# GAP-LAB-CUHK-SZ/GaussReg

Hardware: AMD Instinct MI355X
Metric: GS views/sec @1M pts 640x480 (+ radius_neighbors Mpts/sec, see radius_neighbors) (higher is better)
Workload: dtype f32; 1 GPU; diff_gaussian_rasterization forward: 1000000 synthetic Gaussians (SH deg 3), 640x480, 32 views per step per GPU (configs[1]); gaussians=1000000, width=640, height=480, parallelism=per-view sharding x1

## Files before the change

### gaussreg_amd/csrc/rasterizer.hip

```cpp
#include <algorithm>
#include <type_traits>
#include <vector>

#include <atomic>

#include "raster_shared.hpp"

namespace gr {
namespace {

static_assert(TILE == RASTER_TILE, "get_rect / rect_decode (common.hpp) are written for this tile size");


constexpr int KEY_DEPTH_BITS = 27;
constexpr uint32_t KEY_DEPTH_BASE = 0x3E000000u;

__device__ __forceinline__ uint32_t pack_rect(const int* rmin, const int* rmax) {
  const int w = rmax[0] - rmin[0], h = rmax[1] - rmin[1];
  if (w > 63 || h > 63 || rmin[0] > 126 || rmin[1] > 126) return RECT_MARKER26;
  return (uint32_t)rmin[0] | ((uint32_t)rmin[1] << 7) | ((uint32_t)w << 14) | ((uint32_t)h << 20);
}

constexpr int REC_PLANE = 66;
constexpr int SH_ROW = 13;

template <bool HAS_SH, bool HAS_COV, bool SH16, bool LATE>
__global__ __launch_bounds__(256) void preprocess_kernel(
    int P, int D, int M, int V, const DevView* __restrict__ views, const float* __restrict__ means3D,
    const float* __restrict__ shs, const float* __restrict__ colors_precomp,
    const float* __restrict__ opacities, const float* __restrict__ scales,
    const float* __restrict__ rotations, const float* __restrict__ cov3D_precomp, int W, int H,
    int32_t* __restrict__ radii, float4* __restrict__ rec, uint32_t* __restrict__ dfield,
    uint32_t* __restrict__ rect_raw, int32_t* __restrict__ far_flag, DevView cam1, int far_seq,
    int2* __restrict__ key_mm) {
  if (LATE && blockIdx.x == 0 && threadIdx.x < (int)(sizeof(DevView) / 4))
    reinterpret_cast<float*>(const_cast<DevView*>(views))[threadIdx.x] = reinterpret_cast<const float*>(&cam1)[threadIdx.x];
  __shared__ float4 s_sh[(SH16 && !LATE) ? WAVE * SH_ROW : 1];
  __shared__ float4 s_rec[256 / WAVE][4 * REC_PLANE];
  __shared__ int s_mm[2][2][256 / WAVE];
  int i = blockIdx.x * blockDim.x + threadIdx.x;
  float shr[SH16 ? 48 : 1];
  if (SH16 && !LATE) {
    const int g0 = blockIdx.x * 256;
    const int n_here = min(256, P - g0);
    const float4* src = reinterpret_cast<const float4*>(shs + (int64_t)g0 * 48);
#pragma unroll 1
    for (int w = 0; w < 256 / WAVE; ++w) {
      const int lim = min(WAVE, n_here - w * WAVE) * 12;
#pragma unroll
      for (int u = 0; u < 3; ++u) {
        const int f = threadIdx.x + u * 256;
        if (f < lim) {
          const int g = f / 12, j = f - g * 12;
          s_sh[g * SH_ROW + j] = src[w * WAVE * 12 + f];
        }
      }
      __syncthreads();
      if ((int)threadIdx.x / WAVE == w && i < P) {
#pragma unroll
        for (int j = 0; j < 12; ++j) {
          const float4 t = s_sh[(threadIdx.x & (WAVE - 1)) * SH_ROW + j];
          shr[4 * j] = t.x;
          shr[4 * j + 1] = t.y;
          shr[4 * j + 2] = t.z;
          shr[4 * j + 3] = t.w;
        }
      }
      __syncthreads();
    }
  }
  const bool valid = i < P;
  const int lane = threadIdx.x & (WAVE - 1);
  const int wave_first = i - lane;
  i = min(i, P - 1);
  const float p[3] = {means3D[3 * (int64_t)i], means3D[3 * (int64_t)i + 1], means3D[3 * (int64_t)i + 2]};
  const float opacity = opacities[i];
  float c6[6];
  if (HAS_COV) {
#pragma unroll
    for (int k = 0; k < 6; ++k) c6[k] = cov3D_precomp[6 * (int64_t)i + k];
  }
  const int gx = (W + TILE - 1) / TILE, gy = (H + TILE - 1) / TILE;
  const float* sh = HAS_SH ? shs + (int64_t)i * M * 3 : nullptr;
  float cpre[3] = {0.f, 0.f, 0.f};
  if (!HAS_SH) {
#pragma unroll
    for (int k = 0; k < 3; ++k) cpre[k] = colors_precomp[3 * (int64_t)i + k];
  }
  float4* wrec = s_rec[threadIdx.x / WAVE];
  float mod_prev = 0.f;
  bool have_cov = HAS_COV;
  for (int v = 0; v < V; ++v) {
    const DevView& cam = LATE ? cam1 : views[v];
    const int64_t o = (int64_t)v * P + i;
    int out_radius = 0;
    uint32_t out_field = 0u, out_rect = 0u;
    float out_depth = 0.f, out_sxx = INFINITY, out_syy = INFINITY, out_kc = 0.f;
    float2 out_xy = make_float2(0.f, 0.f);
    float4 out_co = make_float4(0.f, 0.f, 0.f, 0.f);
    bool shade = false;
    float rgb[3] = {0.f, 0.f, 0.f};
    float pv[3];
    xform4x3(cam.view, p, pv);
    if (pv[2] > 0.2f) {
      float ph[4];
      xform4x4(cam.proj, p, ph);
      const float pw = 1.0f / (ph[3] + 0.0000001f);
      const float pprojx = ph[0] * pw, pprojy = ph[1] * pw;
      if (!HAS_COV && (!have_cov || cam.scale_mod != mod_prev)) {
        float sc[3], rot[4];
#pragma unroll
        for (int k = 0; k < 3; ++k) sc[k] = scales[3 * (int64_t)i + k];
#pragma unroll
        for (int k = 0; k < 4; ++k) rot[k] = rotations[4 * (int64_t)i + k];
        cov3d_from_scale_rot(sc, cam.scale_mod, rot, c6);
        have_cov = true;
        mod_prev = cam.scale_mod;
      }
      float cv[3];
      cov2d(pv, cam.fx, cam.fy, cam.tanx, cam.tany, c6, cam.view, cv);
      const float det = cv[0] * cv[2] - cv[1] * cv[1];
      if (det != 0.0f) {
        const float det_inv = 1.f / det;
        const float mid = 0.5f * (cv[0] + cv[2]);
        const float sq = sqrtf(fmaxf(0.1f, mid * mid - det));
        const float l1 = mid + sq, l2 = mid - sq;
        const float my_radius = ceilf(3.f * sqrtf(fmaxf(l1, l2)));
        const float px = ((pprojx + 1.0f) * (float)W - 1.0f) * 0.5f;
        const float py = ((pprojy + 1.0f) * (float)H - 1.0f) * 0.5f;
        int rmin[2], rmax[2];
        get_rect(px, py, (int)my_radius, gx, gy, rmin, rmax);
        const int ntile = (rmax[0] - rmin[0]) * (rmax[1] - rmin[1]);
        if (ntile != 0) {
          shade = true;
          if (HAS_SH && SH16 && LATE) {
            const float4* s4 = reinterpret_cast<const float4*>(shs + (int64_t)i * 48);
#pragma unroll
            for (int jj = 0; jj < 12; ++jj) {
              const float4 t4 = s4[jj];
              shr[4 * jj] = t4.x;
              shr[4 * jj + 1] = t4.y;
              shr[4 * jj + 2] = t4.z;
              shr[4 * jj + 3] = t4.w;
            }
            sh_to_rgb(D, p, cam.campos, [&](int k, int c) { return shr[k * 3 + c]; }, rgb);
          }
          out_depth = pv[2];
          out_radius = (int)my_radius;
          out_xy = make_float2(px, py);
          out_co = make_float4(cv[2] * det_inv, -cv[1] * det_inv, cv[0] * det_inv, opacity);
          const bool cullable = det > 0.0f && l2 >= 0.29f && l1 < 1.0e4f;
          const float kc = cullable ? 1.001f / (0.5f / l1 - 2.0e-6f) : INFINITY;
          out_kc = kc;
          if (cullable) {
            out_sxx = 2.0f * cv[0] * 1.004f;
            out_syy = 2.0f * cv[2] * 1.004f;
            const float pcm = __logf(255.0f * opacity) + 2.0e-3f;
            if (pcm > 0.0f) {
              const float cp = pcm + 2.0e-6f * (pcm * kc);
              const float hx = sqrtf(2.0f * cp * cv[0]) * 1.001f + 1.0e-2f;
              const float hy = sqrtf(2.0f * cp * cv[2]) * 1.001f + 1.0e-2f;
              const float xlo = ceilf(px - hx), xhi = floorf(px + hx), ylo = ceilf(py - hy), yhi = floorf(py + hy);
              if (xlo > -1.0e6f && xhi < 1.0e6f && ylo > -1.0e6f && yhi < 1.0e6f) {
                rmin[0] = max(rmin[0], (int)floorf(xlo / (float)TILE));
                rmin[1] = max(rmin[1], (int)floorf(ylo / (float)TILE));
                rmax[0] = min(rmax[0], (int)floorf(xhi / (float)TILE) + 1);
                rmax[1] = min(rmax[1], (int)floorf(yhi / (float)TILE) + 1);
                if (rmax[0] < rmin[0]) rmax[0] = rmin[0];
                if (rmax[1] < rmin[1]) rmax[1] = rmin[1];
              }
            }
          }
          uint32_t dk = __float_as_uint(out_depth) - KEY_DEPTH_BASE;
          if (dk >= (1u << KEY_DEPTH_BITS)) {
            dk = (1u << KEY_DEPTH_BITS) - 1;
            if (LATE) *far_flag = far_seq; else atomicOr(far_flag, 1);
          }
          out_field = dk;
          out_rect = pack_rect(rmin, rmax);
        }
      }
    }
    if (valid) {
      __builtin_nontemporal_store(out_radius, radii + o);
      dfield[o] = out_field;
      rect_raw[o] = out_rect;
    }
    wrec[0 * REC_PLANE + lane] = make_float4(out_xy.x, out_xy.y, out_sxx, out_syy);
    wrec[1 * REC_PLANE + lane] = out_co;
    wrec[3 * REC_PLANE + lane] = make_float4(__int_as_float(out_radius), out_depth, 0.f, 0.f);
    if (key_mm != nullptr) {
      const uint32_t fld = valid ? out_field : 0u;
      const int mn = wave_min_i32_dpp(fld != 0u ? (int)fld : 0x7fffffff), mx = wave_max_i32_dpp((int)fld);
      if (lane == 0) s_mm[v & 1][0][threadIdx.x / WAVE] = mn, s_mm[v & 1][1][threadIdx.x / WAVE] = mx;
      __syncthreads();
      if (threadIdx.x == 0) {
        int bmn = 0x7fffffff, bmx = 0;
#pragma unroll
        for (int w = 0; w < 256 / WAVE; ++w) bmn = min(bmn, s_mm[v & 1][0][w]), bmx = max(bmx, s_mm[v & 1][1][w]);
        key_mm[(int64_t)v * gridDim.x + blockIdx.x] = make_int2(bmn, bmx);
      }
    }
    if (shade && !(HAS_SH && SH16 && LATE)) {
      if (HAS_SH) {
        if (SH16) sh_to_rgb(D, p, cam.campos, [&](int k, int c) { return shr[k * 3 + c]; }, rgb);
        else sh_to_rgb(D, p, cam.campos, [&](int k, int c) { return sh[k * 3 + c]; }, rgb);
      } else {
        rgb[0] = cpre[0]; rgb[1] = cpre[1]; rgb[2] = cpre[2];
      }
    }
    wrec[2 * REC_PLANE + lane] = make_float4(rgb[0], rgb[1], rgb[2], out_kc);
    const unsigned long long vis = __ballot(valid && out_radius > 0);
    __builtin_amdgcn_fence(__ATOMIC_RELEASE, "wavefront");
    __builtin_amdgcn_wave_barrier();
    __builtin_amdgcn_fence(__ATOMIC_ACQUIRE, "wavefront");
    float4* wout = rec + 4 * ((int64_t)v * P + wave_first);
#pragma unroll
    for (int k = 0; k < 4; ++k) {
      const int rl = 16 * k + lane / 4;
      const float4 piece = wrec[(lane & 3) * REC_PLANE + rl];
      if ((vis >> rl) & 1ull) {
        typedef float pre_f4 __attribute__((ext_vector_type(4)));
        __builtin_nontemporal_store(pre_f4{piece.x, piece.y, piece.z, piece.w}, reinterpret_cast<pre_f4*>(wout + 4 * rl + (lane & 3)));
      }
    }
    __builtin_amdgcn_fence(__ATOMIC_RELEASE, "wavefront");
    __builtin_amdgcn_wave_barrier();
    __builtin_amdgcn_fence(__ATOMIC_ACQUIRE, "wavefront");
  }
}

__global__ __launch_bounds__(256) void full_keys_kernel(int64_t n, const float4* __restrict__ rec,
                                                        const int32_t* __restrict__ radii, uint32_t* __restrict__ dfield) {
  const int64_t o = (int64_t)blockIdx.x * blockDim.x + threadIdx.x;
  if (o >= n) return;
  dfield[o] = radii[o] > 0 ? __float_as_uint(rec[4 * o + 3].y) : 0u;
}


__device__ __forceinline__ bool bin_block(int V, int nchunk, int& v, int& c) {
  const int b = blockIdx.x;
  if (V >= 8) {
    const int k = b >> 3;
    v = (b & 7) + 8 * (k / nchunk);
    c = k % nchunk;
    return v < V;
  }
  v = b / nchunk;
  c = b % nchunk;
  return true;
}
inline int bin_grid(int V, int nchunk) { return V >= 8 ? 8 * ((V + 7) / 8) * nchunk : V * nchunk; }
inline bool bin_scans_self(int nchunk, int V) { return !(nchunk <= SCAN_SINGLE_ROW && V <= 4); }
constexpr int SCATTER_WGS = 6;
constexpr int WIDE_T = 1024;

__device__ __forceinline__ constexpr int mod_small(int n, int d) {
  const unsigned long long tab = d <= 4 ? 0x2001'2aab'4001'8001ull : 0x1001'124a'1556'199aull;
  const unsigned int m = (unsigned int)(tab >> (((d - 1) & 3) * 16)) & 0xffffu;
  return n - (int)(((unsigned int)n * m) >> 15) * d;
}
static_assert(mod_small(255, 7) == 255 % 7 && mod_small(254, 3) == 254 % 3 && mod_small(250, 5) == 0 &&
              mod_small(251, 6) == 251 % 6 && mod_small(255, 8) == 7 && mod_small(200, 1) == 0, "mod_small multipliers");
template <typename F>
__device__ __forceinline__ void by_modulus(int mx, F&& f) {
  switch (mx) {
    case 1: f(std::integral_constant<int, 1>{}); break;
    case 2: f(std::integral_constant<int, 2>{}); break;
    case 3: f(std::integral_constant<int, 3>{}); break;
    case 4: f(std::integral_constant<int, 4>{}); break;
    case 5: f(std::integral_constant<int, 5>{}); break;
    case 6: f(std::integral_constant<int, 6>{}); break;
    case 7: f(std::integral_constant<int, 7>{}); break;
    default: f(std::integral_constant<int, 8>{}); break;
  }
}

__global__ __launch_bounds__(BIN_T) void tile_count_kernel(int P, int V, int gx, int gy, int nchunk,
                                                           const int32_t* __restrict__ nvis,
                                                           const uint32_t* __restrict__ rects,
                                                           const int32_t* __restrict__ ids,
                                                           const float4* __restrict__ rec,
                                                           uint16_t* __restrict__ chunk_cnt,
                                                           int32_t* __restrict__ chunk_total) {
  extern __shared__ unsigned int s_hist[];
  __shared__ int s_wsum[BIN_T / WAVE];
  int v, c;
  if (!bin_block(V, nchunk, v, c)) return;
  const int tiles = gx * gy;
  for (int T = threadIdx.x; T < tiles; T += BIN_T) s_hist[T] = 0u;
  __syncthreads();
  const int64_t vbase = (int64_t)v * P;
  const int nv = nvis[v];
  int mine = 0;
  uint32_t rr[BIN_CHUNK / BIN_T];
#pragma unroll
  for (int it = 0; it < BIN_CHUNK / BIN_T; ++it) {
    const int t = c * BIN_CHUNK + it * BIN_T + threadIdx.x;
    rr[it] = t < nv ? rects[vbase + t] : 0u;
  }
#pragma unroll
  for (int it = 0; it < BIN_CHUNK / BIN_T; ++it) {
    const int t = c * BIN_CHUNK + it * BIN_T + threadIdx.x;
    const uint32_t r = rr[it];
    if (r == 0u) continue;
    int x0, y0, w, h;
    if (!rect_decode(r, r == RECT_MARKER26 ? ids[vbase + t] : 0, vbase, rec, gx, gy, x0, y0, w, h)) continue;
    mine += w * h;
    for (int y = y0; y < y0 + h; ++y)
      for (int x = x0; x < x0 + w; ++x) atomicAdd(&s_hist[y * gx + x], 1u);
  }
  const int wsum = wave_sum_i32_dpp(mine);
  if ((threadIdx.x & (WAVE - 1)) == 0) s_wsum[threadIdx.x / WAVE] = wsum;
  __syncthreads();
  uint16_t* dst = chunk_cnt + ((int64_t)v * nchunk + c) * tiles;
  for (int T = threadIdx.x; T < tiles; T += BIN_T) dst[T] = (uint16_t)s_hist[T];
  if (threadIdx.x == 0) {
    int tot = 0;
    for (int i = 0; i < BIN_T / WAVE; ++i) tot += s_wsum[i];
    chunk_total[v * nchunk + c] = tot;
  }
}

__global__ __launch_bounds__(BIN_T) void chunk_total_kernel(int P, int V, int gx, int gy, int nchunk,
                                                            const int32_t* __restrict__ nvis,
                                                            const uint32_t* __restrict__ rects,
                                                            const int32_t* __restrict__ ids,
                                                            const float4* __restrict__ rec,
                                                            int32_t* __restrict__ chunk_total) {
  __shared__ int s_wsum[BIN_T / WAVE];
  int v, c;
  if (!bin_block(V, nchunk, v, c)) return;
  const int64_t vbase = (int64_t)v * P;
  const int nv = nvis[v];
  int mine = 0;
  uint32_t rr[BIN_CHUNK / BIN_T];
#pragma unroll
  for (int it = 0; it < BIN_CHUNK / BIN_T; ++it) {
    const int t = c * BIN_CHUNK + it * BIN_T + threadIdx.x;
    rr[it] = t < nv ? rects[vbase + t] : 0u;
  }
#pragma unroll
  for (int it = 0; it < BIN_CHUNK / BIN_T; ++it) {
    const int t = c * BIN_CHUNK + it * BIN_T + threadIdx.x;
    const uint32_t r = rr[it];
    int x0, y0, w, h;
    if (r != 0u && rect_decode(r, r == RECT_MARKER26 ? ids[vbase + t] : 0, vbase, rec, gx, gy, x0, y0, w, h)) mine += w * h;
  }
  const int wsum = wave_sum_i32_dpp(mine);
  if ((threadIdx.x & (WAVE - 1)) == 0) s_wsum[threadIdx.x / WAVE] = wsum;
  __syncthreads();
  if (threadIdx.x == 0) {
    int tot = 0;
    for (int i = 0; i < BIN_T / WAVE; ++i) tot += s_wsum[i];
    chunk_total[v * nchunk + c] = tot;
  }
}

__global__ __launch_bounds__(1024) void chunk_max_kernel(int n, const int32_t* __restrict__ chunk_total,
                                                         int32_t* __restrict__ chunk_max) {
  __shared__ int s_m[1024 / WAVE];
  int m = 0;
  for (int i = threadIdx.x; i < n; i += 1024) m = max(m, chunk_total[i]);
  m = wave_max_i32_dpp(m);
  if ((threadIdx.x & (WAVE - 1)) == 0) s_m[threadIdx.x / WAVE] = m;
  __syncthreads();
  if (threadIdx.x == 0) {
    for (int i = 0; i < 1024 / WAVE; ++i) m = max(m, s_m[i]);
    *chunk_max = m;
  }
}

template <bool SELF>
__global__ __launch_bounds__(256) void seg_scan_kernel(int V, int tiles, int nchunk, const uint16_t* __restrict__ chunk_cnt,
                                                       const int32_t* __restrict__ chunk_base ,
                                                       int32_t* __restrict__ totals, uint32_t* __restrict__ seg_off,
                                                       int32_t* __restrict__ mail, int mail_seq) {
  __shared__ int s_w[256 / WAVE];
  __shared__ int s_carry;
  const int v = blockIdx.x / nchunk, c = blockIdx.x % nchunk;
  const int lane = threadIdx.x & (WAVE - 1), wv = threadIdx.x / WAVE;
  int vb = 0;
  if (SELF) {
    const int me = (int)blockIdx.x;
    int part = 0;
    for (int i = threadIdx.x; i < me; i += 256) part += chunk_base[i];
    part = wave_sum_i32_dpp(part);
    if (lane == 0) s_w[wv] = part;
    __syncthreads();
    vb = s_w[0] + s_w[1] + s_w[2] + s_w[3];
    __syncthreads();
    if (c == 0) {
      int sum = 0, mx = 0;
      for (int i = threadIdx.x; i < nchunk; i += 256) {
        const int t = chunk_base[v * nchunk + i];
        sum += t;
        mx = max(mx, t);
      }
      sum = wave_sum_i32_dpp(sum);
      mx = wave_max_i32_dpp(mx);
      if (lane == 0) {
        s_w[wv] = sum;
      }
      __shared__ int s_m[256 / WAVE];
      if (lane == 0) s_m[wv] = mx;
      __syncthreads();
      if (threadIdx.x == 0) {
        const int tv = s_w[0] + s_w[1] + s_w[2] + s_w[3], mv = max(max(s_m[0], s_m[1]), max(s_m[2], s_m[3]));
        totals[v] = tv;
        totals[V + v] = mv;
        if (mail != nullptr) {
          __hip_atomic_store(&mail[v], tv, __ATOMIC_RELAXED, __HIP_MEMORY_SCOPE_SYSTEM);
          __hip_atomic_store(&mail[V + v], mv, __ATOMIC_RELAXED, __HIP_MEMORY_SCOPE_SYSTEM);
          if (v == 0) __hip_atomic_store(&mail[2 * V], totals[2 * V], __ATOMIC_RELAXED, __HIP_MEMORY_SCOPE_SYSTEM);
          __hip_atomic_store(&mail[2 * V + 1 + v], mail_seq, __ATOMIC_RELEASE, __HIP_MEMORY_SCOPE_SYSTEM);
        }
      }
      __syncthreads();
    }
  } else {
    for (int u = 0; u < v; ++u) vb += totals[u];
  }
  const uint16_t* src = chunk_cnt + ((int64_t)v * nchunk + c) * tiles;
  uint32_t* dst = seg_off + ((int64_t)v * nchunk + c) * (tiles + 1);
  if (threadIdx.x == 0) s_carry = SELF ? vb : vb + chunk_base[v * nchunk + c];
  __syncthreads();
  for (int T0 = 0; T0 < tiles; T0 += 256) {
    const int T = T0 + threadIdx.x;
    const int n = T < tiles ? (int)src[T] : 0;
    const int incl = wave_incl_scan_add_dpp(n);
    if (lane == WAVE - 1) s_w[wv] = incl;
    __syncthreads();
    int base = s_carry;
    for (int i = 0; i < wv; ++i) base += s_w[i];
    if (T < tiles) dst[T] = (uint32_t)(base + incl - n);
    __syncthreads();
    if (threadIdx.x == 255) s_carry = base + incl;
    __syncthreads();
  }
  if (threadIdx.x == 0) dst[tiles] = (uint32_t)s_carry;
}

constexpr int SEG_READ = 0, SEG_SELF_RAW = 1, SEG_SELF_SCAN = 2;
struct SelfSeg {
  const int32_t* chunk_total;
  int32_t* totals;
  int32_t* mail;
  int mail_seq;
};
template <bool LANE_ORDERED, int TT, int SEG = SEG_READ>
__global__ __launch_bounds__(TT) void tile_scatter_kernel(int P, int V, int gx, int gy, int nchunk, int tile_bits,
                                                             int stage_cap, const int32_t* __restrict__ nvis,
                                                             const uint32_t* __restrict__ rects,
                                                             const int32_t* __restrict__ ids,
                                                             const float4* __restrict__ rec,
                                                             uint32_t* __restrict__ seg_off,
                                                             int32_t* __restrict__ point_list, unsigned int list_cap, int elist_cap,
                                                             SelfSeg self) {
  extern __shared__ unsigned int s_cur[];
  constexpr int NW = TT / WAVE, CW = BIN_CHUNK / NW;
  constexpr bool SELF = SEG != SEG_READ;
  int v, c;
  if (!bin_block(V, nchunk, v, c)) return;
  const int tiles = gx * gy;
  const int row = (tiles + 1) & ~1;
  uint32_t* seg = seg_off + ((int64_t)v * nchunk + c) * (tiles + 1);
  const int lane = threadIdx.x & (WAVE - 1), wv = threadIdx.x / WAVE;
  const int64_t vbase = (int64_t)v * P;
  const int w_begin = c * BIN_CHUNK + wv * (BIN_CHUNK / (TT / WAVE));
  uint32_t rr[BIN_CHUNK / TT];
  int32_t ii[BIN_CHUNK / TT];
#pragma unroll
  for (int j = 0; j < BIN_CHUNK / TT; ++j) {
    const int64_t o = vbase + min(w_begin + j * WAVE + lane, P - 1);
    rr[j] = rects[o];
    ii[j] = ids[o];
  }
  const int nv = nvis[v];
  __shared__ int s_red[2][TT / WAVE];
  __shared__ unsigned int s_carry;
  unsigned int chunk_begin;
  int total;
  if (SEG == SEG_SELF_RAW) {
    const int me = v * nchunk + c;
    int part = 0;
    for (int i = threadIdx.x; i < me; i += TT) part += self.chunk_total[i];
    part = wave_sum_i32_dpp(part);
    if (lane == 0) s_red[0][wv] = part;
    __syncthreads();
    int front = 0;
#pragma unroll
    for (int w2 = 0; w2 < TT / WAVE; ++w2) front += s_red[0][w2];
    chunk_begin = (unsigned int)front;
    total = self.chunk_total[me];
    if (c == 0) {
      __syncthreads();
      int sum = 0, mx = 0;
      for (int i = threadIdx.x; i < nchunk; i += TT) {
        const int t = self.chunk_total[v * nchunk + i];
        sum += t;
        mx = max(mx, t);
      }
      sum = wave_sum_i32_dpp(sum);
      mx = wave_max_i32_dpp(mx);
      if (lane == 0) s_red[0][wv] = sum, s_red[1][wv] = mx;
      __syncthreads();
      if (threadIdx.x == 0) {
        int tv = 0, mv = 0;
        for (int w2 = 0; w2 < TT / WAVE; ++w2) tv += s_red[0][w2], mv = max(mv, s_red[1][w2]);
        self.totals[v] = tv;
        self.totals[V + v] = mv;
        if (self.mail != nullptr) {
          __hip_atomic_store(&self.mail[v], tv, __ATOMIC_RELAXED, __HIP_MEMORY_SCOPE_SYSTEM);
          __hip_atomic_store(&self.mail[V + v], mv, __ATOMIC_RELAXED, __HIP_MEMORY_SCOPE_SYSTEM);
          if (v == 0) __hip_atomic_store(&self.mail[2 * V], self.totals[2 * V], __ATOMIC_RELAXED, __HIP_MEMORY_SCOPE_SYSTEM);
          __hip_atomic_store(&self.mail[2 * V + 1 + v], self.mail_seq, __ATOMIC_RELEASE, __HIP_MEMORY_SCOPE_SYSTEM);
        }
      }
    }
  } else if (SEG == SEG_SELF_SCAN) {
    unsigned int front = (unsigned int)self.chunk_total[(int64_t)V * nchunk + v * nchunk + c];
    for (int u = 0; u < v; ++u) front += (unsigned int)self.totals[u];
    chunk_begin = front;
    total = self.chunk_total[v * nchunk + c];
  } else {
    chunk_begin = seg[0];
// ... 1216 lines not shown
```

Before: 13270 views/s.

## Double-buffer SH staging, hoist covariance, scalar-load camera, shrink record writes

The SH staging loop in preprocess now double-buffers through the s_sh and s_rec shared buffers and prefetches the next slice into registers, which removes one barrier per slice. The 3D covariance is computed once before the view loop for non-LATE paths. The camera is fetched as wide scalar loads pinned to SGPRs. Shared-memory record writes happen only for visible Gaussians, and the store loop batches its LDS reads before the nontemporal global stores. Together these aim to cut barrier stalls, redundant scale/rotation loads and LDS traffic in the per-view loop. The cost is more register pressure and reliance on invisible lanes' stale LDS slots never being written out, which the visibility ballot masks.

```diff
diff --git a/gaussreg_amd/csrc/rasterizer.hip b/gaussreg_amd/csrc/rasterizer.hip
--- a/gaussreg_amd/csrc/rasterizer.hip
+++ b/gaussreg_amd/csrc/rasterizer.hip
@@ -42,32 +42,36 @@
   float shr[SH16 ? 48 : 1];
   if (SH16 && !LATE) {
     const int g0 = blockIdx.x * 256;
-    const int n_here = min(256, P - g0);
+    const int last = min(256, P - g0) * 12 - 1;
     const float4* src = reinterpret_cast<const float4*>(shs + (int64_t)g0 * 48);
-#pragma unroll 1
-    for (int w = 0; w < 256 / WAVE; ++w) {
-      const int lim = min(WAVE, n_here - w * WAVE) * 12;
-#pragma unroll
-      for (int u = 0; u < 3; ++u) {
-        const int f = threadIdx.x + u * 256;
-        if (f < lim) {
-          const int g = f / 12, j = f - g * 12;
-          s_sh[g * SH_ROW + j] = src[w * WAVE * 12 + f];
-        }
+    const int f0 = threadIdx.x, f1 = threadIdx.x + 256, f2 = threadIdx.x + 512;
+    const int d0 = f0 + f0 / 12, d1 = f1 + f1 / 12, d2 = f2 + f2 / 12;
+    float4* const bufa = reinterpret_cast<float4*>(&s_rec[0][0]);
+    float4 r0 = src[min(f0, last)], r1 = src[min(f1, last)], r2 = src[min(f2, last)];
+    auto slice = [&](auto wc) {
+      constexpr int w = decltype(wc)::value;
+      float4* const b = (w & 1) ? s_sh : bufa;
+      b[d0] = r0, b[d1] = r1, b[d2] = r2;
+      if (w + 1 < 256 / WAVE) {
+        const int o = (w + 1) * WAVE * 12;
+        r0 = src[min(o + f0, last)], r1 = src[min(o + f1, last)], r2 = src[min(o + f2, last)];
       }
       __syncthreads();
-      if ((int)threadIdx.x / WAVE == w && i < P) {
+      if ((int)threadIdx.x / WAVE == w) {
 #pragma unroll
         for (int j = 0; j < 12; ++j) {
-          const float4 t = s_sh[(threadIdx.x & (WAVE - 1)) * SH_ROW + j];
+          const float4 t = b[(threadIdx.x & (WAVE - 1)) * SH_ROW + j];
           shr[4 * j] = t.x;
           shr[4 * j + 1] = t.y;
           shr[4 * j + 2] = t.z;
           shr[4 * j + 3] = t.w;
         }
       }
-      __syncthreads();
-    }
+    };
+    slice(std::integral_constant<int, 0>{});
+    slice(std::integral_constant<int, 1>{});
+    slice(std::integral_constant<int, 2>{});
+    slice(std::integral_constant<int, 3>{});
   }
   const bool valid = i < P;
   const int lane = threadIdx.x & (WAVE - 1);
@@ -90,14 +94,37 @@
   float4* wrec = s_rec[threadIdx.x / WAVE];
   float mod_prev = 0.f;
   bool have_cov = HAS_COV;
+  if (!HAS_COV && !LATE) {
+    float sc[3], rot[4];
+#pragma unroll
+    for (int k = 0; k < 3; ++k) sc[k] = scales[3 * (int64_t)i + k];
+#pragma unroll
+    for (int k = 0; k < 4; ++k) rot[k] = rotations[4 * (int64_t)i + k];
+    mod_prev = views[0].scale_mod;
+    cov3d_from_scale_rot(sc, mod_prev, rot, c6);
+    have_cov = true;
+  }
   for (int v = 0; v < V; ++v) {
-    const DevView& cam = LATE ? cam1 : views[v];
+    typedef uint32_t cam_x16 __attribute__((ext_vector_type(16), aligned(4)));
+    typedef uint32_t cam_x8 __attribute__((ext_vector_type(8), aligned(4)));
+    static_assert(offsetof(DevView, bg) == 160, "the camera without bg is fetched as 16 + 16 + 8 words");
+    DevView cam;
+    if (LATE) {
+      cam = cam1;
+    } else {
+      const uint32_t* cw = reinterpret_cast<const uint32_t*>(views + v);
+      cam_x16 c0 = *reinterpret_cast<const cam_x16*>(cw), c1 = *reinterpret_cast<const cam_x16*>(cw + 16);
+      cam_x8 c2 = *reinterpret_cast<const cam_x8*>(cw + 32);
+      asm volatile("" : "+s"(c0), "+s"(c1), "+s"(c2));
+#pragma unroll
+      for (int k = 0; k < 16; ++k) cam.view[k] = __uint_as_float(c0[k]), cam.proj[k] = __uint_as_float(c1[k]);
+      cam.campos[0] = __uint_as_float(c2[0]), cam.campos[1] = __uint_as_float(c2[1]), cam.campos[2] = __uint_as_float(c2[2]);
+      cam.tanx = __uint_as_float(c2[3]), cam.tany = __uint_as_float(c2[4]);
+      cam.fx = __uint_as_float(c2[5]), cam.fy = __uint_as_float(c2[6]), cam.scale_mod = __uint_as_float(c2[7]);
+    }
     const int64_t o = (int64_t)v * P + i;
     int out_radius = 0;
     uint32_t out_field = 0u, out_rect = 0u;
-    float out_depth = 0.f, out_sxx = INFINITY, out_syy = INFINITY, out_kc = 0.f;
-    float2 out_xy = make_float2(0.f, 0.f);
-    float4 out_co = make_float4(0.f, 0.f, 0.f, 0.f);
     bool shade = false;
     float rgb[3] = {0.f, 0.f, 0.f};
     float pv[3];
@@ -145,13 +172,12 @@
             }
             sh_to_rgb(D, p, cam.campos, [&](int k, int c) { return shr[k * 3 + c]; }, rgb);
           }
-          out_depth = pv[2];
+          const float out_depth = pv[2];
+          float out_sxx = INFINITY, out_syy = INFINITY;
           out_radius = (int)my_radius;
-          out_xy = make_float2(px, py);
-          out_co = make_float4(cv[2] * det_inv, -cv[1] * det_inv, cv[0] * det_inv, opacity);
+          const float4 out_co = make_float4(cv[2] * det_inv, -cv[1] * det_inv, cv[0] * det_inv, opacity);
           const bool cullable = det > 0.0f && l2 >= 0.29f && l1 < 1.0e4f;
           const float kc = cullable ? 1.001f / (0.5f / l1 - 2.0e-6f) : INFINITY;
-          out_kc = kc;
           if (cullable) {
             out_sxx = 2.0f * cv[0] * 1.004f;
             out_syy = 2.0f * cv[2] * 1.004f;
@@ -178,6 +204,11 @@
           }
           out_field = dk;
           out_rect = pack_rect(rmin, rmax);
+          wrec[0 * REC_PLANE + lane] = make_float4(px, py, out_sxx, out_syy);
+          wrec[1 * REC_PLANE + lane] = out_co;
+          wrec[3 * REC_PLANE + lane] = make_float4(__int_as_float(out_radius), out_depth, 0.f, 0.f);
+          if (HAS_SH && SH16 && LATE) wrec[2 * REC_PLANE + lane] = make_float4(rgb[0], rgb[1], rgb[2], kc);
+          else wrec[2 * REC_PLANE + lane].w = kc;
         }
       }
     }
@@ -186,9 +217,6 @@
       dfield[o] = out_field;
       rect_raw[o] = out_rect;
     }
-    wrec[0 * REC_PLANE + lane] = make_float4(out_xy.x, out_xy.y, out_sxx, out_syy);
-    wrec[1 * REC_PLANE + lane] = out_co;
-    wrec[3 * REC_PLANE + lane] = make_float4(__int_as_float(out_radius), out_depth, 0.f, 0.f);
     if (key_mm != nullptr) {
       const uint32_t fld = valid ? out_field : 0u;
       const int mn = wave_min_i32_dpp(fld != 0u ? (int)fld : 0x7fffffff), mx = wave_max_i32_dpp((int)fld);
@@ -208,20 +236,28 @@
       } else {
         rgb[0] = cpre[0]; rgb[1] = cpre[1]; rgb[2] = cpre[2];
       }
-    }
-    wrec[2 * REC_PLANE + lane] = make_float4(rgb[0], rgb[1], rgb[2], out_kc);
+      float4& c4 = wrec[2 * REC_PLANE + lane];
+      c4.x = rgb[0], c4.y = rgb[1], c4.z = rgb[2];
+    }
     const unsigned long long vis = __ballot(valid && out_radius > 0);
     __builtin_amdgcn_fence(__ATOMIC_RELEASE, "wavefront");
     __builtin_amdgcn_wave_barrier();
     __builtin_amdgcn_fence(__ATOMIC_ACQUIRE, "wavefront");
     float4* wout = rec + 4 * ((int64_t)v * P + wave_first);
-#pragma unroll
-    for (int k = 0; k < 4; ++k) {
-      const int rl = 16 * k + lane / 4;
-      const float4 piece = wrec[(lane & 3) * REC_PLANE + rl];
-      if ((vis >> rl) & 1ull) {
-        typedef float pre_f4 __attribute__((ext_vector_type(4)));
-        __builtin_nontemporal_store(pre_f4{piece.x, piece.y, piece.z, piece.w}, reinterpret_cast<pre_f4*>(wout + 4 * rl + (lane & 3)));
+    {
+      typedef float pre_f4 __attribute__((ext_vector_type(4)));
+      pre_f4 piece[4];
+#pragma unroll
+      for (int k = 0; k < 4; ++k) {
+        const float4 t = wrec[(lane & 3) * REC_PLANE + 16 * k + lane / 4];
+        piece[k] = pre_f4{t.x, t.y, t.z, t.w};
+      }
+      asm volatile("" : "+v"(piece[0]), "+v"(piece[1]), "+v"(piece[2]), "+v"(piece[3]));
+      const unsigned long long mine = vis >> (lane / 4);
+#pragma unroll
+      for (int k = 0; k < 4; ++k) {
+        if ((mine >> (16 * k)) & 1ull)
+          __builtin_nontemporal_store(piece[k], reinterpret_cast<pre_f4*>(wout + 4 * (16 * k + lane / 4) + (lane & 3)));
       }
     }
     __builtin_amdgcn_fence(__ATOMIC_RELEASE, "wavefront");
```

After: 13320 views/s (median of 6 runs). About the same (+0.3%).
